# dyouakim/smpl

Measured on AMD Instinct MI355X. Metric: successor evaluations/sec, ManipLattice GetSuccs loop body (7-DOF arm, 256^3 voxel grid), higher is better.
Workload: dtype f64; 1 GPU; cfg2: 7-DOF arm7, 256^3 grid @ 0.02 m, tabletop + 64 boxes (seed 2), frontier batch B=4096 open states x M=25 primitives, eps 5 ARA* frontier; fork semantics (xy rotation by state[3]); batch_states=4096, primitives=25, grid=256, queries=1, parallelism=single query

## Files before the change

### smpl_amd/capi.py

```python
from __future__ import annotations

import ctypes as C
import os

import numpy as np

from . import build as _build

_dp = C.POINTER(C.c_double)
_ip = C.POINTER(C.c_int32)
_up = C.POINTER(C.c_uint8)
_u64p = C.POINTER(C.c_uint64)

SYMBOLS = [
    "smplx_last_error", "smplx_device_count", "smplx_shard_range", "smplx_grid_create", "smplx_grid_destroy", "smplx_model_create",
    "smplx_model_destroy", "smplx_model_counts", "smplx_model_joints", "smplx_model_nodes", "smplx_model_pairs",
    "smplx_space_create", "smplx_space_destroy", "smplx_space_num_vars", "smplx_space_num_prims",
    "smplx_space_discretization", "smplx_cc_state_valid_batch", "smplx_cc_edge_valid_batch", "smplx_cc_interpolate",
    "smplx_cc_sphere_positions", "smplx_set_goal_joint", "smplx_set_goal_xyz", "smplx_goal_pose",
    "smplx_heuristic_batch", "smplx_bfs_size", "smplx_bfs_copy", "smplx_bfs_levels", "smplx_expand_batch",
    "smplx_expand_work_bytes", "smplx_expand_batch_device", "smplx_set_start", "smplx_start_id", "smplx_goal_id",
    "smplx_get_succs", "smplx_hint_frontier", "smplx_get_goal_heuristic", "smplx_num_states", "smplx_get_state",
    "smplx_plan", "smplx_expansion_log_size", "smplx_expansion_log", "smplx_extract_path", "smplx_post_process_path", "smplx_space_specialized", "smplx_model_const_header", "smplx_profile_begin",
    "smplx_profile_end", "smplx_counters_bytes", "smplx_counters_read", "smplx_plan_multi",
# ... 532 lines not shown
        return lib().smplx_num_states(self.h)

    def get_state(self, i):
        q = np.zeros(self.N); c = np.zeros(self.N, np.int32)
        _chk(lib().smplx_get_state(self.h, i, _p(q, _dp), _p(c, _ip)))
        return q, c

    def search_counters(self):
        out = (C.c_int64 * 16)()
        lib().smplx_search_counters.argtypes = [C.c_void_p, C.POINTER(C.c_int64)]
        _chk(lib().smplx_search_counters(self.h, out))
        names = ["searches", "grows", "dup_pushes", "t_idle", "t_select_pop", "t_evaluate", "t_commit", "t_relax", "t_reorder", "t_launch_io",
                 "device_states", "heap_cache_entries", "spec_rounds", "spec_hits"]
        return {n: int(out[i]) for i, n in enumerate(names)}

    def set_search_helper(self, on):
        lib().smplx_test_set_search_helper.argtypes = [C.c_void_p, C.c_int]
        _chk(lib().smplx_test_set_search_helper(self.h, 1 if on else 0))

    def set_pipe_prep(self, on):
        lib().smplx_test_set_pipe_prep.argtypes = [C.c_void_p, C.c_int]
        _chk(lib().smplx_test_set_pipe_prep(self.h, 1 if on else 0))

    def set_search_capacity(self, states):
        lib().smplx_test_set_search_capacity.argtypes = [C.c_void_p, C.c_int]
        _chk(lib().smplx_test_set_search_capacity(self.h, int(states)))

    def plan(self, eps0, eps_final, eps_delta, improve=True, bounded=False, max_init=0, max_rep=0, cap=100000):
        P = SearchParams(eps0, eps_final, eps_delta, int(improve), int(bounded), max_init, max_rep)
        S = SearchStats()
        ids = np.zeros(cap, np.int32)
        _chk(lib().smplx_plan(self.h, C.byref(P), _p(ids, _ip), cap, C.byref(S)))
        n = lib().smplx_expansion_log_size(self.h)
        log = np.zeros(n, np.int32)
        if n:
            _chk(lib().smplx_expansion_log(self.h, _p(log, _ip)))
        out = {f: getattr(S, f) for f, _ in SearchStats._fields_}
        out["path"] = ids[:S.path_len].copy()
        out["expansion_log"] = log
        return out

    @staticmethod
    def plan_multi(spaces, eps0, eps_final, eps_delta, improve=True, bounded=False, max_init=0, max_rep=0, cap=4096,
                   host_threads=1):
        nq = len(spaces)
        P = SearchParams(eps0, eps_final, eps_delta, int(improve), int(bounded), max_init, max_rep)
# ... 75 lines not shown
```

### smpl_amd/csrc/engine.hip

```cpp
#include <hip/hip_runtime.h>

#include <algorithm>
#include <chrono>
#include <cmath>
#include <cstdlib>
#include <cstring>
#include <functional>
#include <limits>
#include <memory>
#include <string>
#include <vector>

#include "../../include/smpl_amd.h"
#include "det_math.h"
#include "device_types.h"
#include "kernels.h"
#include "model_compile.h"
#include "specialize.h"
#include "test_hooks.h"
#include "host_core.h"
#include "grid_handle.h"
#include "lattice.h"
#include "space.h"
#include "bfs_host.h"
// ... 244 lines not shown

    auto bail = [&](hipError_t e, const char* what) {
        const std::string msg = std::string(what) + ": " + hipGetErrorString(e);
        smplx_space_destroy(s);
        return set_error(SMPLX_E_HIP, msg);
    };
    hipError_t e;
    if ((e = hipGetDevice(&s->device)) != hipSuccess) return bail(e, "hipGetDevice");
    if ((e = hipStreamCreate(&s->stream)) != hipSuccess) return bail(e, "hipStreamCreate");
    {
        const char* env = getenv("SMPLX_SPECIALIZE");
        smplx::generic_kernels(s->ks);
        if (params->flags & SMPLX_SPACE_GENERIC_KERNELS) s->specialize_note = "disabled by SMPLX_SPACE_GENERIC_KERNELS";
        else if (env && env[0] == '0') s->specialize_note = "disabled by SMPLX_SPECIALIZE=0";
        else if (!smplx::specialized_kernels(s->model.dev, s->ks, s->specialize_note) && env && env[0] == '2') {
            const std::string msg = "kernel specialisation failed: " + s->specialize_note;
            smplx_space_destroy(s);
            return set_error(SMPLX_E_HIP, msg);
        }
    }
    s->lds_nroot = s->ks.specialized ? 0 : s->model.dev.nroot;
    s->lds_bytes = smplx_lds_bytes(s->blob_bytes, s->lds_nroot, s->model.dev.nslots, s->model.dev.nvars, s->model.dev.stack_bytes);
    s->lds_bytes_valid = smplx_lds_bytes(s->blob_bytes, s->lds_nroot, s->ks.specialized ? 0 : s->model.dev.nslots, s->model.dev.nvars, s->model.dev.stack_bytes);
    if (s->lds_bytes > 160 * 1024) { smplx_space_destroy(s); return set_error(SMPLX_E_LIMIT, "model needs more LDS per block than a CU has (160 KB)"); }
    if ((e = hipEventCreateWithFlags(&s->batch.done, hipEventDisableTiming)) != hipSuccess) return bail(e, "hipEventCreate");
    if ((e = hipMalloc((void**)&s->d_space, sizeof(SmplxSpaceDev))) != hipSuccess) return bail(e, "hipMalloc space");
    const int dx = grid->n[0] + 2, dy = grid->n[1] + 2, dz = grid->n[2] + 2;
    s->bfs.total = (int64_t)dx * dy * dz;
    for (int a = 0; a < 3; ++a) s->bfs.bricks[a] = (grid->n[a] + 7) / 8;
    const size_t nbricks = (size_t)s->bfs.bricks[0] * s->bfs.bricks[1] * s->bfs.bricks[2];
    s->bfs.ints = (int64_t)nbricks * SMPLX_BFS_REC;
    if ((e = hipMalloc((void**)&s->bfs.d_dist, sizeof(int32_t) * s->bfs.ints)) != hipSuccess) return bail(e, "hipMalloc bfs");
    if ((e = hipMalloc((void**)&s->bfs.d_brick_queued, sizeof(int32_t) * 2 * nbricks + 64)) != hipSuccess) return bail(e, "hipMalloc bfs queued");
    if ((e = hipMemset(s->bfs.d_brick_queued, 0, sizeof(int32_t) * 2 * nbricks + 64)) != hipSuccess) return bail(e, "hipMemset bfs queued");
    if ((e = hipMalloc((void**)&s->bfs.d_queue, sizeof(int32_t) * (2 * 16 * nbricks + 64))) != hipSuccess) return bail(e, "hipMalloc bfs queue");
    if ((e = hipMalloc((void**)&s->bfs.d_counts, sizeof(int32_t) * (3 * 16 * 32 + kBfsHistory))) != hipSuccess) return bail(e, "hipMalloc bfs counts");
    s->hs.bfs.dim_x = dx; s->hs.bfs.dim_y = dy; s->hs.bfs.dim_z = dz; s->hs.bfs.dim_xy = dx * dy;
    s->hs.bfs.cost_per_cell = params->cost_per_cell;
    s->hs.bfs.nbx = s->bfs.bricks[0]; s->hs.bfs.nby = s->bfs.bricks[1]; s->hs.bfs.nbz = s->bfs.bricks[2];
    s->hs.bfs.dist = s->bfs.d_dist;
    s->hs.bfs.tag_mask = (int64_t)grid->n[0] * grid->n[1] * grid->n[2] < ((int64_t)1 << 28) ? (int32_t)0xF0000000u : 0;
    s->hs.bfs.tag_word = 0;
    hipLaunchKernelGGL(k_bfs_init, dim3(2048), dim3(256), 0, s->stream, grid->dev, s->bfs.wall_thr, s->bfs.bricks[0], s->bfs.bricks[1], s->bfs.bricks[2], s->bfs.d_dist);
    if ((e = hipGetLastError()) != hipSuccess) return bail(e, "k_bfs_init");
    {
        const char* env = getenv("SMPLX_DEVICE_TABLE");
// ... 25 lines not shown
    if (s->stream) (void)hipStreamDestroy(s->stream);
    delete s;
}

int smplx_space_specialized(const smplx_space* s, char* note, int cap)
{
    if (!s) return 0;
    if (note && cap > 0) { std::strncpy(note, s->specialize_note.c_str(), cap - 1); note[cap - 1] = 0; }
    return s->ks.specialized ? 1 : 0;
}

int smplx_test_set_work_list_items(smplx_space* s, int items)
{
    if (!s || items < 0) return set_error(SMPLX_E_ARG, "bad argument");
    s->step.work_list_items = items / 8 * 8;
    return SMPLX_OK;
}

int smplx_test_set_pipe_prep(smplx_space* s, int on)
{
    if (!s) return set_error(SMPLX_E_ARG, "null space");
    s->step.pipe_prep = on != 0;
    return SMPLX_OK;
}

int smplx_test_set_search_helper(smplx_space* s, int on)
{
    if (!s) return set_error(SMPLX_E_ARG, "null space");
    s->ds.test_no_helper = on == 0;
    return SMPLX_OK;
}

int smplx_test_set_search_capacity(smplx_space* s, int states)
{
    if (!s || states < 0) return set_error(SMPLX_E_ARG, "bad argument");
    s->ds.test_capacity = states;
    return SMPLX_OK;
}

int smplx_search_counters(const smplx_space* s, int64_t out[16])
{
    if (!s || !out) return set_error(SMPLX_E_ARG, "null argument");
    for (int k = 0; k < 16; ++k) out[k] = 0;
    const DevSearch& D = s->ds;
    out[0] = D.searches; out[1] = D.grows; out[2] = D.dup_pushes;
    for (int k = 0; k < 7; ++k) out[3 + k] = D.ticks[k];
// ... 1077 lines not shown
```

### smpl_amd/csrc/kernels.h

```cpp
#pragma once

#ifndef __HIPCC_RTC__
#include <hip/hip_runtime.h>
#include <stdint.h>
#endif

#include "device_types.h"

#define SMPLX_BLOCK 128
#define SMPLX_SETUP_BLOCK (SMPLX_BLOCK + 64)
#define SMPLX_SEARCH_STATIC_LDS (44 * 1024)
#define SMPLX_GLOBAL_AS __attribute__((address_space(1)))
#define SMPLX_TALLIES 6

static inline int smplx_small_block(int nprims) { return ((nprims * 7 + 1) + 63) / 64 * 64 + 64; }
static inline int smplx_search_block(int nprims) { const int b = smplx_small_block(nprims); return b + 64 <= 512 ? b + 64 : b; }
static inline size_t smplx_lds_bytes_n(size_t blob_bytes, int nroot, int nslots, int nvars, int stack_bytes, int nthreads)
{
    return blob_bytes + (size_t)(3 * nroot + 12 * nslots + nvars) * 8 * nthreads + (size_t)stack_bytes * nthreads;
}
static inline size_t smplx_lds_bytes(size_t blob_bytes, int nroot, int nslots, int nvars, int stack_bytes)
{
    return smplx_lds_bytes_n(blob_bytes, nroot, nslots, nvars, stack_bytes, SMPLX_BLOCK);
}

#define SMPLX_PER_ROBOT_KERNELS(X) \
    X(STATE_PREP, k_state_prep) X(EXPAND, k_expand) X(PIPE_PREP, k_pipe_prep) X(PIPE_SETUP, k_pipe_setup) \
    X(PIPE_CONFIGS, k_pipe_configs) X(PIPE_FINISH, k_pipe_finish) X(SMALL_BATCH, k_small_batch) X(EDGE_VALID, k_edge_valid) \
    X(STATE_VALID, k_state_valid) X(HEURISTIC, k_heuristic) X(SPHERE_POSITIONS, k_sphere_positions) X(SEARCH, k_search) \
    X(ATTACHED_POSITIONS, k_attached_positions) X(PLANNING_POSE, k_planning_pose)

extern "C" {
__global__ void k_state_prep(const SmplxSpaceDev* S, const double* Q, int B, double* goal_dist,
                             unsigned char* parent_valid, int* parent_lookups,
                         const SmplxSpaceDev* const* stab, const unsigned short* state_q);
__global__ void k_expand(const SmplxSpaceDev* S, const double* Q, int B, const double* goal_dist,
                         const unsigned char* parent_valid, const int* parent_lookups, unsigned char* out_flags,
                         int* out_coord, double* out_q, int* out_h, int* out_cost, int* out_lookups,
                         unsigned long long* counters, const int* deferred_count,
                         const SmplxSpaceDev* const* stab, const unsigned short* state_q);
__global__ void k_pipe_prep(const SmplxSpaceDev* S, const double* Q, int B, double* goal_dist,
                            int* work_count,
                         const SmplxSpaceDev* const* stab, const unsigned short* state_q, int* cmp_totals,
                            const int* ins_items, int n_ins, double* trig);
__global__ void k_pipe_setup(const SmplxSpaceDev* S, const double* Q, int B, double* goal_dist,
                             unsigned char* out_flags, double* out_q, int* edge_w, int* edge_lookups,
                             unsigned char* edge_bad, int* state_lookups, unsigned char* state_bad, unsigned long long* work,
                             int* work_count, int capacity,
                         const SmplxSpaceDev* const* stab, const unsigned short* state_q, int have_goal_dist,
                             int* cmp_totals, const int* ins_items, int n_ins, int nprims, int nvars, double* trig);
__global__ void k_pipe_configs(const SmplxSpaceDev* S, const double* Q, int B, const double* out_q,
                               const int* edge_w, int* edge_lookups, unsigned char* edge_bad, int* state_lookups,
                               unsigned char* state_bad, const unsigned long long* work, const int* work_count, int capacity,
                               int cfg_blocks, const unsigned char* out_flags, int* succ_coord,
                         const SmplxSpaceDev* const* stab, const unsigned short* state_q, int want_id,
                               unsigned long long* succ_eval, unsigned char* succ_goal, int nprims, int nvars,
                               const unsigned char* blob, int blob_bytes, const double* trig);
__global__ void k_pipe_finish(const SmplxSpaceDev* S, const double* Q, int B, const int* edge_w,
                              const int* edge_lookups, const unsigned char* edge_bad, const int* state_lookups,
                              const unsigned char* state_bad, unsigned char* out_flags, int* out_coord, double* out_q,
                              int* out_h, int* out_cost, int* out_lookups, unsigned long long* counters,
                              const double* goal_dist,
                         const SmplxSpaceDev* const* stab, const unsigned short* state_q, int* out_id, SmplxCompactDev cmp,
                              const unsigned long long* succ_eval, const unsigned char* succ_goal, const int* succ_coord,
                              int* work_count, int nprims, int nvars);
__global__ void k_small_batch(const SmplxSpaceDev* S, const double* Q, int B, double* goal_dist_out,
                              unsigned char* state_bad_out, int* state_lookups_out, unsigned char* out_flags, int* out_coord,
                              double* out_q, int* out_h, int* out_cost, int* out_lookups,
                              const SmplxSpaceDev* const* stab, const unsigned short* state_q, unsigned char* host_flags,
                              int* host_coord, double* host_q, int* host_h, int* out_id, int* host_id, const int* ins_items,
                              int n_ins);
__global__ void k_search(const SmplxSpaceDev* const* stab, int max_steps, int lh, int* status_out, long long pre_ticks);
__global__ void k_search_table_fill(const SmplxSpaceDev* Sq, const int* coord, int first, int n, int nvars);
__global__ void k_heap_ops(const int* ops, int nops, int lh, unsigned long long* heap_hbm, SmplxSState* st, int* top_after);
__global__ void k_edge_valid(const SmplxSpaceDev* S, const double* Aq, const double* Bq, int n, unsigned char* out,
                             int* out_lookups, int* out_waypoints);
__global__ void k_state_valid(const SmplxSpaceDev* S, const double* Q, int n, unsigned char* out, int* out_lookups);
__global__ void k_heuristic(const SmplxSpaceDev* S, const double* Q, int n, int* out_h, double* out_xyz);
__global__ void k_planning_pose(const SmplxSpaceDev* S, const double* Q, int n, double* out_T);
__global__ void k_sphere_positions(const SmplxSpaceDev* S, const double* Q, int n, double* out);
__global__ void k_attached_positions(const SmplxSpaceDev* S, const double* Q, int n, double* out);
__global__ void k_table_insert(const SmplxSpaceDev* S, const SmplxSpaceDev* const* stab, const int* items, int n, int nvars);
__global__ void k_bfs_metric(SmplxGridDev grid, SmplxBfsDev bfs, const double* xyz, int n, double* out);
__global__ void k_bfs_init(SmplxGridDev g, int wall_thr, int nbx, int nby, int nbz, int* dist);
__global__ void k_bfs_reset(int* dist, size_t total);
__global__ void k_bfs_export(SmplxBfsDev b, int* out);
__global__ void k_bfs_brick_seed(int* dist, int cx, int cy, int cz, int nbx, int nby, int nbz, int* list0, int* counts, int tag_word);
__global__ void k_bfs_brick_wave(int* dist, int nbx, int nby, int nbz, const int* list_in, const int* counts_in, int* list_next,
// ... 5 lines not shown
```

### smpl_amd/csrc/kernels.hip

```cpp
#ifndef __HIPCC_RTC__
#include <hip/hip_runtime.h>
#endif

#include "kernels.h"

#define BLOCK SMPLX_BLOCK

#include "bfs_record.h"
#include "model_lds.h"
#include "sphere_checks.h"
#include "attached_bodies.h"
#include "config_checks.h"
#include "lattice_steps.h"
#include "step_kernels.h"
#include "small_batch.h"
#include "query_kernels.h"
#include "bfs_kernels.h"
#include "search_kernel.h"
```

### smpl_amd/csrc/space.h

```cpp
#pragma once

#include <chrono>
#include <cstdint>
#include <memory>
#include <string>
#include <utility>
#include <vector>

#include "device_types.h"
#include "grid_handle.h"
#include "host_core.h"
#include "lattice.h"
#include "model_compile.h"
#include "specialize.h"

namespace {

struct OutView {
    double* sq = nullptr;
    int32_t* coord = nullptr;
    int32_t* h = nullptr;
    int32_t* id = nullptr;
    unsigned char* flags = nullptr;
    size_t bytes = 0;
// ... 54 lines not shown

struct PlainSpeculation {
    bool plain_mode = false;
    int auto_spec = 96;
    double auto_w = 5.0;
    std::vector<std::pair<uint64_t, int32_t>> pool;
    std::vector<int32_t> hint;
};

struct SmallBatchGovernor {
    int batch_max = 512;
    double latency_limit = 70e-6;
    bool adaptive = false;
    double latency = 0.0;
    int seen = 0, pipeline_left = 0;
    int64_t small_launches = 0, pipe_launches = 0;
};

struct StepLaunch {
    bool fused_mode = false;
    int work_list_items = 0;
    bool pipe_prep = false;
    int three_launch_blocks = 0;
    struct WorkCounters { hipStream_t stream; int32_t* p; bool dirty; };
    std::vector<WorkCounters> work_counters;
    std::vector<hipEvent_t> prof_events;
    size_t prof_used = 0;
};

struct AttachedBodies {
    struct Body {
        std::string id, link;
        int joint = -1;
        std::vector<double> xyzr;
        std::vector<std::string> allowed;
        int first = 0, count = 0;
    };
    std::vector<Body> bodies;
    SmplxBodiesDev* d_bodies = nullptr;
    uint64_t epoch = 0;
    uint64_t epoch_goal = 0;
};

const char* const kBodiesChanged = "bodies were attached or detached after the goal was set: cached successors are stale, set the goal again";

struct Search;
// ... 107 lines not shown
```

### smpl_amd/csrc/step.h

```cpp
#pragma once

#include <algorithm>
#include <chrono>
#include <cstddef>
#include <cstdlib>
#include <cstring>
#include <functional>
#include <string>
#include <utility>
#include <vector>

#include "device_table.h"
#include "kernels.h"
#include "space.h"

namespace {

inline size_t counter_words(int B, int M) { return (size_t)blocks_for((long long)B * M, SMPLX_BLOCK) * SMPLX_TALLIES; }

struct ExpandWork {
    double* goal_dist;
    int32_t* state_lookups;
    unsigned char* state_bad;
    int32_t* edge_w;
// ... 56 lines not shown
    int32_t* h = nullptr;
    int32_t* id = nullptr;
};

struct ExpandArgs {
    const double* q = nullptr;
    int B = 0;
    unsigned char* flags = nullptr;
    int32_t* coord = nullptr;
    double* sq = nullptr;
    int32_t* h = nullptr;
    int32_t* cost = nullptr;
    int32_t* lookups = nullptr;
    void* work = nullptr;
    unsigned long long* counters = nullptr;
    hipStream_t stream = nullptr;
    const SmplxSpaceDev* const* stab = nullptr;
    const unsigned short* state_q = nullptr;
    const ZeroCopy* zero_copy = nullptr;
    const K5Out* k5 = nullptr;
    bool force_pipeline = false;
};

enum class ExpandPath { SmallZeroCopy, Small, Fused, Pipeline };

inline size_t small_lds_bytes(const smplx_space* s)
{
    return smplx_lds_bytes_n(s->blob_bytes, s->lds_nroot, s->model.dev.nslots, s->model.dev.nvars, s->model.dev.stack_bytes,
                             smplx_small_block(s->M));
}

ExpandPath expand_path(const smplx_space* s, int B, int zero_copy_max, bool force_pipeline)
{
    const bool small = !s->step.fused_mode && B <= s->small.batch_max && smplx_small_block(s->M) <= 512 &&
                       small_lds_bytes(s) <= 150 * 1024 && s->step.work_list_items == 0 && s->small.pipeline_left == 0 &&
                       s->step.prof_used + 3 > s->step.prof_events.size();
    if (small && B <= zero_copy_max && s->step.prof_events.empty()) return ExpandPath::SmallZeroCopy;
    if (small && !force_pipeline) return ExpandPath::Small;
    return s->step.fused_mode ? ExpandPath::Fused : ExpandPath::Pipeline;
}

int work_counters_for(smplx_space* s, hipStream_t stream, StepLaunch::WorkCounters** out)
{
    for (StepLaunch::WorkCounters& w : s->step.work_counters)
        if (w.stream == stream) { *out = &w; return SMPLX_OK; }
    int32_t* p = nullptr;
    HIP_TRY(hipMalloc((void**)&p, 2048));
    hipError_t e = hipMemsetAsync(p, 0, 2048, stream);
    if (e == hipSuccess) e = hipStreamSynchronize(stream);
    if (e != hipSuccess) { (void)hipFree(p); return set_error(SMPLX_E_HIP, std::string("work-list counters: ") + hipGetErrorString(e)); }
    s->step.work_counters.push_back({stream, p, false});
    *out = &s->step.work_counters.back();
    return SMPLX_OK;
}

int launch_expand(smplx_space* s, const ExpandArgs& a)
{
    const int B = a.B;
    ExpandWork k = carve_work(a.work, B, s->M, s->N);
    int32_t* d_id = a.k5 ? a.k5->d_id : nullptr;
    SmplxCompactDev cmp;
    std::memset(&cmp, 0, sizeof(cmp));
    if (a.k5 && a.k5->cmp) cmp = *a.k5->cmp;
    const ExpandPath path = expand_path(s, B, a.zero_copy ? B : 0, a.force_pipeline || cmp.rec_a);
    const int32_t* ins_items = a.k5 && s->dt.d_table ? a.k5->items : nullptr;
    const int n_ins = ins_items ? a.k5->n_items : 0;
    if (s->step.work_list_items > 0) k.capacity = s->step.work_list_items;
    hipEvent_t* ev = nullptr;
    if (s->step.prof_used + 3 <= s->step.prof_events.size()) { ev = &s->step.prof_events[s->step.prof_used]; s->step.prof_used += 3; }
    const int bs = blocks_for(B, SMPLX_BLOCK);
    const int be = blocks_for((long long)B * s->M, SMPLX_BLOCK);
    if (path == ExpandPath::SmallZeroCopy || path == ExpandPath::Small) {
        ++s->small.small_launches;
        const ZeroCopy* zc = path == ExpandPath::SmallZeroCopy ? a.zero_copy : nullptr;
        const int small_block = smplx_small_block(s->M);
        KLAUNCH(s, K_SMALL_BATCH, k_small_batch, dim3(B + blocks_for(n_ins, small_block)), dim3(small_block), small_lds_bytes(s), a.stream, s->d_space,
                           zc ? zc->q : a.q, B, k.goal_dist,
                           k.state_bad, k.state_lookups, a.flags, a.coord, a.sq, a.h, a.cost, a.lookups, a.stab, a.state_q,
                           zc ? zc->flags : (unsigned char*)nullptr, zc ? zc->coord : (int32_t*)nullptr,
                           zc ? zc->sq : (double*)nullptr, zc ? zc->h : (int32_t*)nullptr, d_id,
                           zc ? zc->id : (int32_t*)nullptr, ins_items, n_ins);
    } else if (path == ExpandPath::Fused) {
        if (d_id) HIP_TRY(hipMemsetAsync(d_id, 0xFF, sizeof(int32_t) * (size_t)B * s->M, a.stream));
        if (n_ins > 0) {
            hipLaunchKernelGGL(k_table_insert, dim3(blocks_for(n_ins, SMPLX_BLOCK)), dim3(SMPLX_BLOCK), 0, a.stream, s->d_space, a.stab, ins_items, n_ins, s->N);
        }
        if (ev) (void)hipEventRecord(ev[0], a.stream);
        KLAUNCH(s, K_STATE_PREP, k_state_prep, dim3(bs), dim3(SMPLX_BLOCK), s->lds_bytes, a.stream, s->d_space, a.q, B,
                           k.goal_dist, k.state_bad, k.state_lookups, a.stab, a.state_q);
        if (ev) (void)hipEventRecord(ev[1], a.stream);
        KLAUNCH(s, K_EXPAND, k_expand, dim3(be), dim3(SMPLX_BLOCK), s->lds_bytes, a.stream, s->d_space, a.q, B,
                           k.goal_dist, k.state_bad, k.state_lookups, a.flags, a.coord, a.sq, a.h, a.cost, a.lookups,
                           a.counters, (const int*)nullptr, a.stab, a.state_q);
        if (ev) (void)hipEventRecord(ev[2], a.stream);
    } else {
        const size_t lm = s->blob_bytes;
        ++s->small.pipe_launches;
        StepLaunch::WorkCounters* wc = nullptr;
        if (int e = work_counters_for(s, a.stream, &wc)) return e;
        if (wc->dirty) HIP_TRY(hipMemsetAsync(wc->p, 0, 2048, a.stream));
        wc->dirty = true;
        k.work_count = wc->p;
        if (s->step.three_launch_blocks == 0) {
            int cus = 0;
            if (hipDeviceGetAttribute(&cus, hipDeviceAttributeMultiprocessorCount, s->device) != hipSuccess || cus <= 0) cus = 256;
            s->step.three_launch_blocks = cus * 4 * 4 / (SMPLX_SETUP_BLOCK / 64);
        }
        const bool pipe_prep = s->step.pipe_prep || be > s->step.three_launch_blocks;
        if (pipe_prep)
            KLAUNCH(s, K_PIPE_PREP, k_pipe_prep, dim3(bs + blocks_for(n_ins, SMPLX_BLOCK)), dim3(SMPLX_BLOCK), lm, a.stream, s->d_space, a.q, B,
                               k.goal_dist, k.work_count, a.stab, a.state_q, cmp.totals, ins_items, n_ins, k.trig);
        const int n_ins_setup = pipe_prep ? 0 : n_ins;
        KLAUNCH(s, K_PIPE_SETUP, k_pipe_setup, dim3(be + blocks_for(n_ins_setup, SMPLX_BLOCK)), dim3(pipe_prep ? SMPLX_BLOCK : SMPLX_SETUP_BLOCK), lm, a.stream, s->d_space, a.q, B,
                           k.goal_dist, a.flags, a.sq, k.edge_w, k.edge_lookups, k.edge_bad, k.state_lookups, k.state_bad,
                           k.work, k.work_count, k.capacity, a.stab, a.state_q, pipe_prep ? 1 : 0, cmp.totals, ins_items, n_ins_setup,
                           s->M, s->N, k.trig);
        if (ev) (void)hipEventRecord(ev[0], a.stream);
        const int bc = blocks_for((long long)B + (long long)B * s->M * 3, SMPLX_BLOCK);
        const unsigned char* blob = reinterpret_cast<const unsigned char*>(s->d_space) + offsetof(SmplxSpaceDev, model_blob);
        KLAUNCH(s, K_PIPE_CONFIGS, k_pipe_configs, dim3(bc + be), dim3(SMPLX_BLOCK), s->lds_bytes_valid, a.stream, s->d_space, a.q, B,
                           a.sq, k.edge_w, k.edge_lookups, k.edge_bad, k.state_lookups, k.state_bad, k.work, k.work_count,
                           k.capacity, bc, a.flags, k.succ_coord, a.stab, a.state_q, d_id ? 1 : 0, k.succ_eval, k.succ_goal,
                           s->M, s->N, blob, (int)s->blob_bytes, k.trig);
// ... 302 lines not shown
```

### smpl_amd/csrc/step_kernels.h

```cpp
#pragma once

#include "config_checks.h"
#include "lattice_steps.h"


extern "C" __global__ void __launch_bounds__(BLOCK, 2)
k_state_prep(const SmplxSpaceDev* __restrict__ S, const double* __restrict__ Q, int B,
             double* __restrict__ goal_dist, unsigned char* __restrict__ parent_valid, int* __restrict__ parent_lookups,
        const SmplxSpaceDev* const* __restrict__ stab, const unsigned short* __restrict__ state_q)
{
    extern __shared__ __align__(16) unsigned char smem[];
    ModelLds Mv;
    ThreadLds L = setup_lds(S, smem, &Mv);
    const ModelLds* M = &Mv;
    const SmplxGridDev grid = S->grid;
    const int i = blockIdx.x * BLOCK + threadIdx.x;
    if (i >= B) return;
    const SmplxBfsDev bfs = (stab ? stab[state_q[i]] : S)->bfs;
    const double* q = Q + (int64_t)i * MV_NVARS(M);
    goal_dist[i] = metric_goal_distance(M, grid, bfs, q);
    EdgeRef e;
    e.start = q; e.finish = q; e.alpha = 0.0;
    int lk = 0;
    const bool ok = config_valid(M, L, grid, e, lk);
    parent_valid[i] = ok ? 1 : 0;
    parent_lookups[i] = lk;
}

__device__ __forceinline__ void tally_block(unsigned long long* __restrict__ counters, int ev, int va, int lk, int pf,
                                            int cfgs, int slk)
{
    __shared__ int t_acc[BLOCK / 64][SMPLX_TALLIES];
    const int wv = threadIdx.x >> 6;
    for (int off = 32; off > 0; off >>= 1) {
        lk += __shfl_down(lk, off); pf += __shfl_down(pf, off); cfgs += __shfl_down(cfgs, off); slk += __shfl_down(slk, off);
    }
    if ((threadIdx.x & 63) == 0) {
        t_acc[wv][0] = ev; t_acc[wv][1] = va; t_acc[wv][2] = lk; t_acc[wv][3] = pf; t_acc[wv][4] = cfgs; t_acc[wv][5] = slk;
    }
    __syncthreads();
    if (threadIdx.x < SMPLX_TALLIES) {
        int v = 0;
#pragma unroll
        for (int k = 0; k < BLOCK / 64; ++k) v += t_acc[k][threadIdx.x];
        counters[(size_t)blockIdx.x * SMPLX_TALLIES + threadIdx.x] += (unsigned long long)v;
    }
}

struct EdgeTally { int flags, lookups, performed, evaluated; };

__device__ __forceinline__ EdgeTally expand_edge(const ModelLds* __restrict__ M, const ThreadLds& L, const SmplxSpaceDev* __restrict__ S,
                                                 const SmplxSpaceDev* __restrict__ Sq, const SmplxGridDev& grid,
                                                 const double* __restrict__ Q, long long tid,
                                                 const double* __restrict__ goal_dist, bool parent_ok, int parent_lk,
                                                 unsigned char* __restrict__ out_flags, int* __restrict__ out_coord,
                                                 double* __restrict__ out_q, int* __restrict__ out_h, int* __restrict__ out_cost,
                                                 int* __restrict__ out_lookups)
{
    const SmplxActionsDev& A = S->actions;
    const int nprims = A.nprims;
    int flags = SMPLX_F_INACTIVE;
    int lookups = 0;
    int performed = 0;
    int evaluated = 0;
    {
        const int si = (int)(tid / nprims);
        const int pi = (int)(tid - (long long)si * nprims);
// ... 627 lines not shown
```

Before: 1.688 billion successor evaluations/s.

## Add single-kernel block-local expansion step replacing multi-launch pipeline

Adds k_step_block, which does state prep, edge value computation, config collision checks, successor output and compaction for a block of edges in one launch. Parent states covered by a block are checked inside that block, and a last-block-done counter finalises the compaction totals. The path is picked automatically when the model is specialised, at least four blocks fit per CU, and the grid fits in the resident block count. The aim is to remove per-step launch overhead and the global round trips between the pipeline's stages. In exchange, states that straddle two blocks are checked twice, the block uses more LDS, and the work counter buffer grows.

```diff
diff --git a/smpl_amd/capi.py b/smpl_amd/capi.py
--- a/smpl_amd/capi.py
+++ b/smpl_amd/capi.py
@@ -578,6 +578,22 @@
         lib().smplx_test_set_pipe_prep.argtypes = [C.c_void_p, C.c_int]
         _chk(lib().smplx_test_set_pipe_prep(self.h, 1 if on else 0))
 
+    def set_one_launch(self, mode):
+        lib().smplx_test_set_one_launch.argtypes = [C.c_void_p, C.c_int]
+        _chk(lib().smplx_test_set_one_launch(self.h, int(mode)))
+
+    def one_launch_steps(self):
+        lib().smplx_test_one_launch_steps.argtypes = [C.c_void_p]
+        lib().smplx_test_one_launch_steps.restype = C.c_longlong
+        return int(lib().smplx_test_one_launch_steps(self.h))
+
+    def step_counters_zero(self, stream=None):
+        lib().smplx_test_step_counters_zero.argtypes = [C.c_void_p, C.c_void_p]
+        r = lib().smplx_test_step_counters_zero(self.h, C.c_void_p(stream))
+        if r < 0:
+            _chk(r)
+        return r == 1
+
     def set_search_capacity(self, states):
         lib().smplx_test_set_search_capacity.argtypes = [C.c_void_p, C.c_int]
         _chk(lib().smplx_test_set_search_capacity(self.h, int(states)))
diff --git a/smpl_amd/csrc/engine.hip b/smpl_amd/csrc/engine.hip
--- a/smpl_amd/csrc/engine.hip
+++ b/smpl_amd/csrc/engine.hip
@@ -290,6 +290,9 @@
     s->lds_nroot = s->ks.specialized ? 0 : s->model.dev.nroot;
     s->lds_bytes = smplx_lds_bytes(s->blob_bytes, s->lds_nroot, s->model.dev.nslots, s->model.dev.nvars, s->model.dev.stack_bytes);
     s->lds_bytes_valid = smplx_lds_bytes(s->blob_bytes, s->lds_nroot, s->ks.specialized ? 0 : s->model.dev.nslots, s->model.dev.nvars, s->model.dev.stack_bytes);
+    s->step.one_launch_lds = smplx_lds_bytes_n(s->blob_bytes, s->lds_nroot, s->ks.specialized ? 0 : s->model.dev.nslots, s->model.dev.nvars,
+                                               s->model.dev.stack_bytes, SMPLX_STEP_BLOCK);
+    s->step.one_launch_blocks = step_block_resident(s, s->step.one_launch_lds, &s->step.one_launch_per_cu);
     if (s->lds_bytes > 160 * 1024) { smplx_space_destroy(s); return set_error(SMPLX_E_LIMIT, "model needs more LDS per block than a CU has (160 KB)"); }
     if ((e = hipEventCreateWithFlags(&s->batch.done, hipEventDisableTiming)) != hipSuccess) return bail(e, "hipEventCreate");
     if ((e = hipMalloc((void**)&s->d_space, sizeof(SmplxSpaceDev))) != hipSuccess) return bail(e, "hipMalloc space");
@@ -361,6 +364,29 @@
     if (!s) return set_error(SMPLX_E_ARG, "null space");
     s->step.pipe_prep = on != 0;
     return SMPLX_OK;
+}
+
+int smplx_test_set_one_launch(smplx_space* s, int mode)
+{
+    if (!s || mode < -1 || mode > 1) return set_error(SMPLX_E_ARG, "bad argument");
+    s->step.one_launch = mode;
+    return SMPLX_OK;
+}
+
+long long smplx_test_one_launch_steps(const smplx_space* s) { return s ? (long long)s->step.one_launch_steps : -1; }
+
+int smplx_test_step_counters_zero(smplx_space* s, void* stream)
+{
+    if (!s) return set_error(SMPLX_E_ARG, "null space");
+    for (StepLaunch::WorkCounters& w : s->step.work_counters) {
+        if (w.stream != (hipStream_t)stream) continue;
+        std::vector<int32_t> h(SMPLX_WORK_COUNTER_BYTES / sizeof(int32_t));
+        HIP_TRY(hipStreamSynchronize(w.stream));
+        HIP_TRY(hipMemcpy(h.data(), w.p, SMPLX_WORK_COUNTER_BYTES, hipMemcpyDeviceToHost));
+        for (int32_t v : h) if (v != 0) return 0;
+        return 1;
+    }
+    return set_error(SMPLX_E_ARG, "no step has run on this stream");
 }
 
 int smplx_test_set_search_helper(smplx_space* s, int on)
diff --git a/smpl_amd/csrc/kernels.h b/smpl_amd/csrc/kernels.h
--- a/smpl_amd/csrc/kernels.h
+++ b/smpl_amd/csrc/kernels.h
@@ -9,6 +9,12 @@
 
 #define SMPLX_BLOCK 128
 #define SMPLX_SETUP_BLOCK (SMPLX_BLOCK + 64)
+#define SMPLX_STEP_BLOCK SMPLX_SETUP_BLOCK
+#define SMPLX_STEP_STATES 16
+#define SMPLX_STEP_CTR_BASE 512
+#define SMPLX_STEP_CTR_OVERFLOW (SMPLX_STEP_CTR_BASE + 64 * SMPLX_CMP_SHARDS)
+#define SMPLX_STEP_CTR_DONE (SMPLX_STEP_CTR_OVERFLOW + 32)
+#define SMPLX_WORK_COUNTER_BYTES 16384
 #define SMPLX_SEARCH_STATIC_LDS (44 * 1024)
 #define SMPLX_GLOBAL_AS __attribute__((address_space(1)))
 #define SMPLX_TALLIES 6
@@ -24,11 +30,13 @@
     return smplx_lds_bytes_n(blob_bytes, nroot, nslots, nvars, stack_bytes, SMPLX_BLOCK);
 }
 
+static inline int smplx_step_states(int nprims) { return (SMPLX_BLOCK - 2 + nprims) / nprims + 1; }
+
 #define SMPLX_PER_ROBOT_KERNELS(X) \
     X(STATE_PREP, k_state_prep) X(EXPAND, k_expand) X(PIPE_PREP, k_pipe_prep) X(PIPE_SETUP, k_pipe_setup) \
     X(PIPE_CONFIGS, k_pipe_configs) X(PIPE_FINISH, k_pipe_finish) X(SMALL_BATCH, k_small_batch) X(EDGE_VALID, k_edge_valid) \
     X(STATE_VALID, k_state_valid) X(HEURISTIC, k_heuristic) X(SPHERE_POSITIONS, k_sphere_positions) X(SEARCH, k_search) \
-    X(ATTACHED_POSITIONS, k_attached_positions) X(PLANNING_POSE, k_planning_pose)
+    X(ATTACHED_POSITIONS, k_attached_positions) X(PLANNING_POSE, k_planning_pose) X(STEP_BLOCK, k_step_block)
 
 extern "C" {
 __global__ void k_state_prep(const SmplxSpaceDev* S, const double* Q, int B, double* goal_dist,
@@ -64,6 +72,10 @@
                          const SmplxSpaceDev* const* stab, const unsigned short* state_q, int* out_id, SmplxCompactDev cmp,
                               const unsigned long long* succ_eval, const unsigned char* succ_goal, const int* succ_coord,
                               int* work_count, int nprims, int nvars);
+__global__ void k_step_block(const SmplxSpaceDev* S, const double* Q, int B, unsigned char* out_flags, int* out_coord,
+                             double* out_q, int* out_h, int* out_cost, int* out_lookups, unsigned long long* counters,
+                             const SmplxSpaceDev* const* stab, const unsigned short* state_q, int* out_id, SmplxCompactDev cmp,
+                             int* step_ctr, int nprims, int nvars, const unsigned char* blob, int blob_bytes);
 __global__ void k_small_batch(const SmplxSpaceDev* S, const double* Q, int B, double* goal_dist_out,
                               unsigned char* state_bad_out, int* state_lookups_out, unsigned char* out_flags, int* out_coord,
                               double* out_q, int* out_h, int* out_cost, int* out_lookups,
diff --git a/smpl_amd/csrc/kernels.hip b/smpl_amd/csrc/kernels.hip
--- a/smpl_amd/csrc/kernels.hip
+++ b/smpl_amd/csrc/kernels.hip
@@ -13,6 +13,7 @@
 #include "config_checks.h"
 #include "lattice_steps.h"
 #include "step_kernels.h"
+#include "step_block.h"
 #include "small_batch.h"
 #include "query_kernels.h"
 #include "bfs_kernels.h"
diff --git a/smpl_amd/csrc/space.h b/smpl_amd/csrc/space.h
--- a/smpl_amd/csrc/space.h
+++ b/smpl_amd/csrc/space.h
@@ -100,6 +100,11 @@
     int work_list_items = 0;
     bool pipe_prep = false;
     int three_launch_blocks = 0;
+    int one_launch = -1;
+    size_t one_launch_lds = 0;
+    int one_launch_per_cu = 0;
+    int one_launch_blocks = 0;
+    int64_t one_launch_steps = 0;
     struct WorkCounters { hipStream_t stream; int32_t* p; bool dirty; };
     std::vector<WorkCounters> work_counters;
     std::vector<hipEvent_t> prof_events;
diff --git a/smpl_amd/csrc/step.h b/smpl_amd/csrc/step.h
--- a/smpl_amd/csrc/step.h
+++ b/smpl_amd/csrc/step.h
@@ -102,7 +102,7 @@
     bool force_pipeline = false;
 };
 
-enum class ExpandPath { SmallZeroCopy, Small, Fused, Pipeline };
+enum class ExpandPath { SmallZeroCopy, Small, Fused, Pipeline, OneLaunch };
 
 inline size_t small_lds_bytes(const smplx_space* s)
 {
@@ -117,7 +117,27 @@
                        s->step.prof_used + 3 > s->step.prof_events.size();
     if (small && B <= zero_copy_max && s->step.prof_events.empty()) return ExpandPath::SmallZeroCopy;
     if (small && !force_pipeline) return ExpandPath::Small;
-    return s->step.fused_mode ? ExpandPath::Fused : ExpandPath::Pipeline;
+    if (s->step.fused_mode) return ExpandPath::Fused;
+    const bool can_run = s->step.one_launch_blocks > 0 && !s->step.pipe_prep && s->step.work_list_items == 0 &&
+                         s->step.prof_used + 3 > s->step.prof_events.size();
+    const bool by_rule = s->ks.specialized && s->step.one_launch_per_cu >= 4 &&
+                         blocks_for((long long)B * s->M, SMPLX_BLOCK) <= s->step.one_launch_blocks;
+    if (can_run && s->step.one_launch != 0 && (s->step.one_launch == 1 || by_rule)) return ExpandPath::OneLaunch;
+    return ExpandPath::Pipeline;
+}
+
+int step_block_resident(const smplx_space* s, size_t lds, int* blocks_per_cu)
+{
+    *blocks_per_cu = 0;
+    if (smplx_step_states(s->M) > SMPLX_STEP_STATES) return 0;
+    int per_cu = 0, cus = 0;
+    const smplx::KernelRef& k = s->ks.k[smplx::K_STEP_BLOCK];
+    const hipError_t e = k.fn ? hipModuleOccupancyMaxActiveBlocksPerMultiprocessor(&per_cu, k.fn, SMPLX_STEP_BLOCK, lds)
+                              : hipOccupancyMaxActiveBlocksPerMultiprocessor(&per_cu, k.generic, SMPLX_STEP_BLOCK, lds);
+    if (e != hipSuccess) { (void)hipGetLastError(); return 0; }
+    if (hipDeviceGetAttribute(&cus, hipDeviceAttributeMultiprocessorCount, s->device) != hipSuccess || cus <= 0) cus = 256;
+    *blocks_per_cu = per_cu > 0 ? per_cu : 0;
+    return per_cu > 0 ? per_cu * cus : 0;
 }
 
 int work_counters_for(smplx_space* s, hipStream_t stream, StepLaunch::WorkCounters** out)
@@ -125,8 +145,8 @@
     for (StepLaunch::WorkCounters& w : s->step.work_counters)
         if (w.stream == stream) { *out = &w; return SMPLX_OK; }
     int32_t* p = nullptr;
-    HIP_TRY(hipMalloc((void**)&p, 2048));
-    hipError_t e = hipMemsetAsync(p, 0, 2048, stream);
+    HIP_TRY(hipMalloc((void**)&p, SMPLX_WORK_COUNTER_BYTES));
+    hipError_t e = hipMemsetAsync(p, 0, SMPLX_WORK_COUNTER_BYTES, stream);
     if (e == hipSuccess) e = hipStreamSynchronize(stream);
     if (e != hipSuccess) { (void)hipFree(p); return set_error(SMPLX_E_HIP, std::string("work-list counters: ") + hipGetErrorString(e)); }
     s->step.work_counters.push_back({stream, p, false});
@@ -143,6 +163,9 @@
     std::memset(&cmp, 0, sizeof(cmp));
     if (a.k5 && a.k5->cmp) cmp = *a.k5->cmp;
     const ExpandPath path = expand_path(s, B, a.zero_copy ? B : 0, a.force_pipeline || cmp.rec_a);
+    if (s->step.one_launch == 1 && path == ExpandPath::Pipeline)
+        return set_error(SMPLX_E_ARG, "the one-launch step was asked for (smplx_test_set_one_launch) but cannot run: a pipeline test hook or a "
+                                      "profile-event triple is set, or a block of k_step_block does not fit this model");
     const int32_t* ins_items = a.k5 && s->dt.d_table ? a.k5->items : nullptr;
     const int n_ins = ins_items ? a.k5->n_items : 0;
     if (s->step.work_list_items > 0) k.capacity = s->step.work_list_items;
@@ -173,12 +196,27 @@
                            k.goal_dist, k.state_bad, k.state_lookups, a.flags, a.coord, a.sq, a.h, a.cost, a.lookups,
                            a.counters, (const int*)nullptr, a.stab, a.state_q);
         if (ev) (void)hipEventRecord(ev[2], a.stream);
+    } else if (path == ExpandPath::OneLaunch) {
+        ++s->small.pipe_launches;
+        StepLaunch::WorkCounters* wc = nullptr;
+        if (int e = work_counters_for(s, a.stream, &wc)) return e;
+        if (wc->dirty) HIP_TRY(hipMemsetAsync(wc->p, 0, SMPLX_WORK_COUNTER_BYTES, a.stream));
+        wc->dirty = true;
+        if (n_ins > 0) {
+            hipLaunchKernelGGL(k_table_insert, dim3(blocks_for(n_ins, SMPLX_BLOCK)), dim3(SMPLX_BLOCK), 0, a.stream, s->d_space, a.stab, ins_items, n_ins, s->N);
+        }
+        const unsigned char* blob = reinterpret_cast<const unsigned char*>(s->d_space) + offsetof(SmplxSpaceDev, model_blob);
+        KLAUNCH(s, K_STEP_BLOCK, k_step_block, dim3(be), dim3(SMPLX_STEP_BLOCK), s->step.one_launch_lds, a.stream, s->d_space, a.q, B,
+                           a.flags, a.coord, a.sq, a.h, a.cost, a.lookups, a.counters, a.stab, a.state_q, d_id, cmp, wc->p,
+                           s->M, s->N, blob, (int)s->blob_bytes);
+        wc->dirty = false;
+        ++s->step.one_launch_steps;
     } else {
         const size_t lm = s->blob_bytes;
         ++s->small.pipe_launches;
         StepLaunch::WorkCounters* wc = nullptr;
         if (int e = work_counters_for(s, a.stream, &wc)) return e;
-        if (wc->dirty) HIP_TRY(hipMemsetAsync(wc->p, 0, 2048, a.stream));
+        if (wc->dirty) HIP_TRY(hipMemsetAsync(wc->p, 0, SMPLX_WORK_COUNTER_BYTES, a.stream));
         wc->dirty = true;
         k.work_count = wc->p;
         if (s->step.three_launch_blocks == 0) {
diff --git a/smpl_amd/csrc/step_block.h b/smpl_amd/csrc/step_block.h
--- /dev/null
+++ b/smpl_amd/csrc/step_block.h
@@ -0,0 +1,349 @@
+#pragma once
+
+#include "step_kernels.h"
+
+extern "C" __global__ void __launch_bounds__(SMPLX_STEP_BLOCK)
+k_step_block(const SmplxSpaceDev* __restrict__ S, const double* __restrict__ Q, int B,
+             unsigned char* __restrict__ out_flags, int* out_coord, double* out_q,
+             int* __restrict__ out_h, int* __restrict__ out_cost, int* __restrict__ out_lookups,
+             unsigned long long* __restrict__ counters,
+        const SmplxSpaceDev* const* __restrict__ stab, const unsigned short* __restrict__ state_q,
+             int* __restrict__ out_id, SmplxCompactDev cmp, int* __restrict__ step_ctr, int nprims, int nvars,
+             const unsigned char* __restrict__ blob, int blob_bytes)
+{
+    extern __shared__ __align__(16) unsigned char smem[];
+    constexpr int NT = SMPLX_STEP_BLOCK;
+#ifdef SMPLX_CONST_MODEL
+    constexpr bool RS = true;
+#else
+    constexpr bool RS = false;
+#endif
+    __shared__ double s_gd[SMPLX_STEP_STATES];
+    __shared__ int s_slk[SMPLX_STEP_STATES], s_sbad[SMPLX_STEP_STATES];
+    __shared__ int s_W[BLOCK], s_pre[BLOCK], s_elk[BLOCK], s_ebad[BLOCK];
+    __shared__ int s_wsum[BLOCK / 64];
+#ifdef SMPLX_CONST_MODEL
+    __shared__ double s_sq[CM_NV * BLOCK];
+    __shared__ double s_pq[SMPLX_STEP_STATES * CM_NV];
+    __shared__ double s_trig[CM_PARENT_TRIG ? SMPLX_STEP_STATES * SMPLX_TRIG_ROW : 1];
+#endif
+    const int t = (int)threadIdx.x;
+    const ModelFetch fetched = model_fetch(blob, blob_bytes, NT);
+    const SmplxActionsDev& A = S->actions;
+    const int nv = ARG_NVARS(nvars);
+    const long long n_edges = (long long)B * nprims;
+    const long long e0 = (long long)blockIdx.x * BLOCK;
+    const long long e1 = e0 + BLOCK - 1 < n_edges ? e0 + BLOCK - 1 : n_edges - 1;
+    const int s0 = (int)(e0 / nprims), s1 = (int)(e1 / nprims);
+    const int n_states = s1 - s0 + 1;
+    const bool dist_wave = t >= BLOCK;
+    const int l = t - BLOCK;
+    const long long tid = e0 + t;
+    const bool in_range = !dist_wave && tid < n_edges;
+    const int si = in_range ? (int)(tid / nprims) : s0;
+    const int pi = in_range ? (int)(tid - (long long)si * nprims) : 0;
+    const int ks = si - s0;
+    const SmplxSpaceDev* Sq = stab ? stab[state_q[si]] : S;
+    const int type = A.type[pi];
+    if (t < BLOCK) { s_elk[t] = 0; s_ebad[t] = 0; }
+    if (t < SMPLX_STEP_STATES) { s_slk[t] = 0; s_sbad[t] = 0; }
+#ifdef SMPLX_CONST_MODEL
+    double pqv[CM_NV], sqv[CM_NV];
+#pragma unroll
+    for (int v = 0; v < CM_NV; ++v) { pqv[v] = 0.0; sqv[v] = 0.0; }
+    if (in_range) {
+#pragma unroll
+        for (int v = 0; v < CM_NV; ++v) pqv[v] = Q[(int64_t)si * CM_NV + v];
+    }
+    for (int i = t; i < n_states * CM_NV; i += NT) s_pq[i] = Q[(int64_t)s0 * CM_NV + i];
+#endif
+    ModelLds Mv;
+    ThreadLds L = setup_lds(S, smem, &Mv, NT, !RS, blob, blob_bytes, fetched);
+    const ModelLds* M = &Mv;
+    const SmplxGridDev grid = S->grid;
+    int W = 0;
+    int flags = SMPLX_F_INACTIVE;
+    int succ_h = 0, succ_id = -1;
+    bool succ_goal = false;
+#ifdef SMPLX_CONST_MODEL
+    int scv[CM_NV];
+#pragma unroll
+    for (int v = 0; v < CM_NV; ++v) scv[v] = 0;
+    if (in_range) flags = pipe_edge_values(M, A, Sq, pi, pqv, sqv, W);
+    if (dist_wave) {
+        if constexpr (CM_PARENT_TRIG) {
+            constexpr int PER = 64 / CM_NV;
+            const int ls = l / CM_NV, lv = l - ls * CM_NV;
+            for (int r0 = 0; r0 < n_states; r0 += PER) {
+                const int k = r0 + ls;
+                double ns = 0.0, nc = 0.0;
+                if (ls < PER && k < n_states) {
+                    const double x = s_pq[k * CM_NV + lv];
+                    double rs = 0.0, rc = 0.0;
+                    if ((CM_TRIG_ANY >> lv) & 1u) smplx_sincos(x, &rs, &rc);
+                    ns = rs; nc = rc;
+                    bool cont = false;
+#pragma unroll
+                    for (int u = 0; u < CM_NV; ++u) if (CM_VAR_TYPE[u] == SMPLX_JT_CONTINUOUS) cont = cont || lv == u;
+                    if (cont && ((CM_TRIG_ANY >> lv) & 1u)) {
+                        const double xn = smplx_normalize_angle(x);
+                        if (__double_as_longlong(xn) != __double_as_longlong(x)) smplx_sincos(xn, &ns, &nc);
+                    }
+                    double* row = s_trig + k * SMPLX_TRIG_ROW;
+                    row[2 * lv] = rs; row[2 * lv + 1] = rc;
+                    row[2 * CM_NV + 2 * lv] = ns; row[2 * CM_NV + 2 * lv + 1] = nc;
+                }
+                double sn[CM_NV], cs[CM_NV];
+#pragma unroll
+                for (int v = 0; v < CM_NV; ++v) {
+                    const int from = (l * CM_NV + v) & 63;
+                    sn[v] = __shfl(ns, from); cs[v] = __shfl(nc, from);
+                }
+                if (l < PER && r0 + l < n_states) {
+                    const int k2 = r0 + l;
+                    const SmplxBfsDev bfs = (stab ? stab[state_q[s0 + k2]] : S)->bfs;
+                    double qd[CM_NV];
+#pragma unroll
+                    for (int v = 0; v < CM_NV; ++v) qd[v] = s_pq[k2 * CM_NV + v];
+                    s_gd[k2] = metric_goal_distance_sc(M, grid, bfs, qd, sn, cs);
+                }
+            }
+        } else if (l < n_states) {
+            const SmplxBfsDev bfs = (stab ? stab[state_q[s0 + l]] : S)->bfs;
+            double qd[CM_NV];
+#pragma unroll
+            for (int v = 0; v < CM_NV; ++v) qd[v] = s_pq[l * CM_NV + v];
+            s_gd[l] = metric_goal_distance(M, grid, bfs, qd);
+        }
+    }
+#else
+    if (dist_wave && l < n_states) {
+        const SmplxBfsDev bfs = (stab ? stab[state_q[s0 + l]] : S)->bfs;
+        s_gd[l] = metric_goal_distance(M, grid, bfs, Q + (int64_t)(s0 + l) * nv);
+    }
+#endif
+    __syncthreads();
+    int items = 0;
+    if (in_range) {
+        if (!mprim_active(A, s_gd[ks], type)) {
+            flags = SMPLX_F_INACTIVE;
+            W = 0;
+        } else {
+#ifdef SMPLX_CONST_MODEL
+            if (flags != SMPLX_F_INACTIVE) {
+#pragma unroll
+                for (int v = 0; v < CM_NV; ++v) { s_sq[v * BLOCK + t] = sqv[v]; out_q[tid * CM_NV + v] = sqv[v]; }
+            }
+#ifndef ABL_NO_SUCC
+            if (flags == 0) {
+                constexpr bool SC = CM_PARENT_TRIG && CM_TRIG_PLANNING != 0;
+                if constexpr (SC) {
+                    double prow[2 * CM_NV], sn[CM_NV], cs[CM_NV];
+#pragma unroll
+                    for (int j = 0; j < 2 * CM_NV; ++j) prow[j] = s_trig[ks * SMPLX_TRIG_ROW + 2 * CM_NV + j];
+                    parent_trig<CM_TRIG_PLANNING, true>(sqv, pqv, prow, sn, cs);
+                    pipe_successor<true>(M, Sq, grid, sqv, scv, out_id != nullptr, succ_h, succ_id, succ_goal, sn, cs);
+                } else {
+                    pipe_successor(M, Sq, grid, sqv, scv, out_id != nullptr, succ_h, succ_id, succ_goal);
+                }
+            }
+#endif
+#else
+            flags = pipe_edge_values(M, A, Sq, pi, Q + (int64_t)si * nv, out_q + tid * nv, W);
+#endif
+        }
+        items = W > 0 ? W - 1 : 0;
+    }
+    const int lane = t & 63, wv = t >> 6;
+    int incl = items;
+    for (int off = 1; off < 64; off <<= 1) {
+        const int u = __shfl_up(incl, off);
+        if (lane >= off) incl += u;
+    }
+    if (!dist_wave) {
+        s_W[t] = W;
+        s_pre[t] = incl;
+        if (lane == 63) s_wsum[wv] = incl;
+    }
+    __syncthreads();
+    {
+        int wave_first[BLOCK / 64 + 1];
+        wave_first[0] = 0;
+#pragma unroll
+        for (int k = 0; k < BLOCK / 64; ++k) wave_first[k + 1] = wave_first[k] + s_wsum[k];
+        const int total = n_states + wave_first[BLOCK / 64];
+        for (int i = t; i < total; i += NT) {
+            const bool is_state = i < n_states;
+            int k = i, edge = 0, wp = 0, Wi = 0;
+            if (!is_state) {
+                int j = i - n_states;
+                int w = 0;
+#pragma unroll
+                for (int u = 1; u < BLOCK / 64; ++u) w += (j >= wave_first[u]) ? 1 : 0;
+                j -= wave_first[w];
+                int lo = 0;
+#pragma unroll
+                for (int step = 32; step > 0; step >>= 1)
+                    if (s_pre[w * 64 + lo + step - 1] <= j) lo += step;
+                edge = w * 64 + lo;
+                Wi = s_W[edge];
+                wp = j - (s_pre[edge] - (Wi - 1)) + 1;
+                k = (int)((e0 + edge) / nprims) - s0;
+            }
+            EdgeRef e;
+            e.alpha = is_state ? 0.0 : (double)wp * (1.0 / (double)(Wi - 1));
+            int lk = 0;
+            bool ok;
+#ifdef SMPLX_CONST_MODEL
+            e.start = nullptr; e.finish = nullptr;
+            constexpr bool SC = CM_PARENT_TRIG;
+            double qs[CM_NV], qc[CM_NV], prow[2 * CM_NV];
+#pragma unroll
+            for (int v = 0; v < CM_NV; ++v) { qs[v] = s_pq[k * CM_NV + v]; qc[v] = qs[v]; }
+            if constexpr (SC) {
+#pragma unroll
+                for (int j = 0; j < 2 * CM_NV; ++j) prow[j] = s_trig[k * SMPLX_TRIG_ROW + j];
+            }
+#ifndef ABL_NO_FK
+#pragma unroll
+            for (int v = 0; v < CM_NV; ++v) {
+                const double sv = qs[v];
+                double q = sv;
+                if (e.alpha != 0.0) q = sv + e.alpha * edge_diff(M, v, sv, s_sq[v * BLOCK + edge]);
+                lds_d(L, L.q_base + v) = q;
+                qc[v] = q;
+            }
+#endif
+            if constexpr (SC) {
+                double sn[CM_NV], cs[CM_NV];
+                parent_trig<CM_TRIG_COLLISION, false>(qc, qs, prow, sn, cs);
+                ok = config_valid_staged<RS, true>(M, L, grid, e, lk, sn, cs);
+            } else {
+                ok = config_valid_staged<RS>(M, L, grid, e, lk);
+            }
+#else
+            e.start = Q + (int64_t)(s0 + k) * nv;
+            e.finish = is_state ? e.start : out_q + (e0 + edge) * nv;
+            ok = config_valid<RS>(M, L, grid, e, lk);
+#endif
+            if (is_state) {
+                s_slk[k] = lk;
+                if (!ok) s_sbad[k] = 1;
+            } else {
+                atomicAdd(&s_elk[edge], lk);
+                if (!ok) s_ebad[edge] = 1;
+            }
+        }
+    }
+    __syncthreads();
+    int lookups = 0, performed = 0, evaluated = 0, ncfg = 0, slk = 0;
+    if (in_range) {
+        const int s_lk = s_slk[ks];
+        if (pi == 0) { slk = s_lk; ncfg = 1; }
+        int h = 0, cost = 0;
+        if (!(flags & SMPLX_F_INACTIVE)) evaluated = 1;
+        if (flags == 0) {
+            if (W > 0) ncfg += W - 1;
+            performed = s_elk[t];
+            const bool ok = (W == 0) || (s_sbad[ks] == 0 && s_ebad[t] == 0);
+            lookups = performed + (W > 0 ? s_lk : 0);
+            if (!ok) {
+                flags = SMPLX_F_COLLISION;
+                succ_id = -1;
+            } else {
+#ifdef SMPLX_CONST_MODEL
+#pragma unroll
+                for (int v = 0; v < CM_NV; ++v) out_coord[tid * CM_NV + v] = scv[v];
+#else
+                pipe_successor(M, Sq, grid, out_q + tid * nv, out_coord + tid * nv, out_id != nullptr, succ_h, succ_id, succ_goal);
+#endif
+                h = succ_h;
+                cost = A.cost[pi];
+                flags = SMPLX_F_VALID | (succ_goal ? SMPLX_F_GOAL : 0);
+            }
+        } else {
+            succ_id = -1;
+        }
+        out_flags[tid] = (unsigned char)flags;
+        out_h[tid] = h;
+        out_cost[tid] = cost;
+        out_lookups[tid] = lookups;
+        succ_h = h;
+        if (out_id) out_id[tid] = succ_id;
+    }
+    if (cmp.rec_a) {
+        __shared__ int c_cnt[BLOCK / 64][2];
+        __shared__ int c_base[2];
+        const bool is_a = in_range && (flags & SMPLX_F_VALID) != 0;
+        const bool is_b = is_a && (succ_id < 0 || (flags & SMPLX_F_GOAL) != 0);
+        const unsigned long long m_a = __ballot(is_a), m_b = __ballot(is_b);
+        const unsigned long long below = lane == 0 ? 0ull : (~0ull >> (64 - lane));
+        if (lane == 0 && !dist_wave) { c_cnt[wv][0] = __popcll(m_a); c_cnt[wv][1] = __popcll(m_b); }
+        __syncthreads();
+        if (t == 0) {
+            int ta = 0, tb = 0;
+#pragma unroll
+            for (int k = 0; k < BLOCK / 64; ++k) { ta += c_cnt[k][0]; tb += c_cnt[k][1]; }
+            const int shard = blockIdx.x % SMPLX_CMP_SHARDS;
+            const int sa = cmp.cap_a / SMPLX_CMP_SHARDS, sb = cmp.cap_b / SMPLX_CMP_SHARDS;
+            int ba = ta > 0 ? atomicAdd(&step_ctr[SMPLX_STEP_CTR_BASE + 64 * shard], ta) : 0;
+            int bb = tb > 0 ? atomicAdd(&step_ctr[SMPLX_STEP_CTR_BASE + 64 * shard + 32], tb) : 0;
+            if (ba + ta > sa || bb + tb > sb) {
+                atomicExch(&step_ctr[SMPLX_STEP_CTR_OVERFLOW], 1);
+                __threadfence();
+                ba = -1;
+            }
+            else { ba += shard * sa; bb += shard * sb; }
+            c_base[0] = ba; c_base[1] = bb;
+            int* bt = cmp.block_tab + 4 * (size_t)blockIdx.x;
+            bt[0] = ba; bt[1] = ta; bt[2] = bb; bt[3] = tb;
+        }
+        __syncthreads();
+        if (c_base[0] >= 0 && is_a) {
+            int ia = c_base[0] + __popcll(m_a & below), ib = c_base[1] + __popcll(m_b & below);
+            for (int k = 0; k < wv; ++k) { ia += c_cnt[k][0]; ib += c_cnt[k][1]; }
+            cmp.rec_a[2 * (size_t)ia] = succ_id;
+            cmp.rec_a[2 * (size_t)ia + 1] = pi | ((flags & SMPLX_F_GOAL) ? 0x100 : 0) | (si << 9);
+            if (is_b) {
+                unsigned char* rb = cmp.rec_b + (size_t)ib * cmp.rec_b_bytes;
+                int* ri = (int*)rb;
+                double* rq = (double*)(rb + (size_t)((nv + 2) / 2 * 2) * 4);
+                ri[0] = succ_h;
+#ifdef SMPLX_CONST_MODEL
+#pragma unroll
+                for (int v = 0; v < CM_NV; ++v) { ri[1 + v] = scv[v]; rq[v] = s_sq[v * BLOCK + t]; }
+#else
+                for (int v = 0; v < nv; ++v) { ri[1 + v] = out_coord[tid * nv + v]; rq[v] = out_q[tid * nv + v]; }
+#endif
+            }
+        }
+    }
+    if (counters) {
+        const unsigned long long m_eval = __ballot(evaluated);
+        const unsigned long long m_valid = __ballot((flags & SMPLX_F_VALID) != 0);
+        tally_block<NT / 64>(counters, dist_wave ? 0 : __popcll(m_eval), dist_wave ? 0 : __popcll(m_valid), lookups, performed, ncfg, slk);
+    }
+    if (cmp.rec_a) {
+        __shared__ int s_last;
+        if (t == 0) {
+            const int nb = (int)gridDim.x, shard = blockIdx.x % SMPLX_CMP_SHARDS;
+            const int in_shard = (nb - shard + SMPLX_CMP_SHARDS - 1) / SMPLX_CMP_SHARDS;
+            const int shards = nb < SMPLX_CMP_SHARDS ? nb : SMPLX_CMP_SHARDS;
+            int last = 0;
+            if (atomicAdd(&step_ctr[SMPLX_STEP_CTR_DONE + 32 * (1 + shard)], 1) == in_shard - 1)
+                last = atomicAdd(&step_ctr[SMPLX_STEP_CTR_DONE], 1) == shards - 1 ? 1 : 0;
+            s_last = last;
+        }
+        __syncthreads();
+        if (s_last) {
+            if (t < 2 * SMPLX_CMP_SHARDS) {
+                const int shard = t >> 1, region = t & 1;
+                cmp.totals[32 * shard + region] = atomicExch(&step_ctr[SMPLX_STEP_CTR_BASE + 64 * shard + 32 * region], 0);
+            } else if (t == 2 * SMPLX_CMP_SHARDS) {
+                cmp.totals[32 * SMPLX_CMP_SHARDS] = atomicExch(&step_ctr[SMPLX_STEP_CTR_OVERFLOW], 0);
+            } else if (t <= 2 * SMPLX_CMP_SHARDS + 1 + SMPLX_CMP_SHARDS) {
+                atomicExch(&step_ctr[SMPLX_STEP_CTR_DONE + 32 * (t - 2 * SMPLX_CMP_SHARDS - 1)], 0);
+            }
+        }
+    }
+}
diff --git a/smpl_amd/csrc/step_kernels.h b/smpl_amd/csrc/step_kernels.h
--- a/smpl_amd/csrc/step_kernels.h
+++ b/smpl_amd/csrc/step_kernels.h
@@ -27,10 +27,11 @@
     parent_lookups[i] = lk;
 }
 
+template <int WAVES = BLOCK / 64>
 __device__ __forceinline__ void tally_block(unsigned long long* __restrict__ counters, int ev, int va, int lk, int pf,
                                             int cfgs, int slk)
 {
-    __shared__ int t_acc[BLOCK / 64][SMPLX_TALLIES];
+    __shared__ int t_acc[WAVES][SMPLX_TALLIES];
     const int wv = threadIdx.x >> 6;
     for (int off = 32; off > 0; off >>= 1) {
         lk += __shfl_down(lk, off); pf += __shfl_down(pf, off); cfgs += __shfl_down(cfgs, off); slk += __shfl_down(slk, off);
@@ -42,7 +43,7 @@
     if (threadIdx.x < SMPLX_TALLIES) {
         int v = 0;
 #pragma unroll
-        for (int k = 0; k < BLOCK / 64; ++k) v += t_acc[k][threadIdx.x];
+        for (int k = 0; k < WAVES; ++k) v += t_acc[k][threadIdx.x];
         counters[(size_t)blockIdx.x * SMPLX_TALLIES + threadIdx.x] += (unsigned long long)v;
     }
 }
```

Result: faster. 1.939 billion successor evaluations/s (median of 6 runs) (+14.8%).
